# tkonolige/city2ba

Measured on AMD Instinct MI355X. Metric: million observations/sec (project+Jacobian), higher is better.
Workload: dtype f64

## Files before the change

city2ba_amd/csrc/camera_math.hpp:

```cpp
#pragma once
#include <hip/hip_runtime.h>
#include <stdint.h>
#include "pow4_libm.hpp"

namespace c2b {

#define C2B_DEV __device__ __forceinline__

constexpr int kCamBlk = 32;
constexpr int kCamHot = 24;
constexpr int kR = 0, kT = 9, kIntr = 12, kJl = 15, kCenter = 24;

constexpr int kCamGroup = 8;
__host__ __device__ inline int cam_in_group_at(int k, int j) {
    return j < 16 ? k * 16 + j : (j < 24 ? 128 + k * 8 + (j - 16) : (j < 28 ? 192 + k * 4 + (j - 24) : 224 + k * 4 + (j - 28)));
}
__host__ __device__ inline int64_t cam_group_at(int64_t c) { return (c >> 3) * (int64_t)(kCamGroup * kCamBlk); }
__host__ __device__ inline int64_t cam_light_at(int64_t c) { return cam_group_at(c) + (c & 7) * 16; }
__host__ __device__ inline int64_t cam_center_at(int64_t c) { return cam_group_at(c) + 192 + (c & 7) * 4; }
__host__ __device__ inline int64_t cam_at(int64_t c, int j) { return cam_group_at(c) + cam_in_group_at((int)(c & 7), j); }
__host__ __device__ inline int64_t cam_chunk_at(int64_t c, int j2) { return cam_at(c, 2 * j2); }
__host__ __device__ inline int64_t cam_table_doubles(int64_t n_cam) { return ((n_cam + kCamGroup - 1) / kCamGroup * kCamGroup) * (int64_t)kCamBlk; }
struct CamRec {
    const double *group; int k;
// ... 27 lines not shown
        for (int r = 0; r < 3; ++r)
            o[3 * c + r] = dot3(a[r], a[3 + r], a[6 + r], b[3 * c], b[3 * c + 1], b[3 * c + 2]);
}

template <typename T>
C2B_DEV void cm_center(const T *m, T tx, T ty, T tz, T c[3]) {
    const T m00 = m[0], m01 = m[1], m02 = m[2];
    const T m10 = m[3], m11 = m[4], m12 = m[5];
    const T m20 = m[6], m21 = m[7], m22 = m[8];
    const T det = m00 * (m11 * m22 - m21 * m12) - m10 * (m01 * m22 - m21 * m02) +
                  m20 * (m01 * m12 - m11 * m02);
    const T a0 = (m11 * m22 - m12 * m21) / det, a1 = (m12 * m20 - m10 * m22) / det,
            a2 = (m10 * m21 - m11 * m20) / det;
    const T b0 = (m21 * m02 - m22 * m01) / det, b1 = (m22 * m00 - m20 * m02) / det,
            b2 = (m20 * m01 - m21 * m00) / det;
    const T c0 = (m01 * m12 - m02 * m11) / det, c1 = (m02 * m10 - m00 * m12) / det,
            c2 = (m00 * m11 - m01 * m10) / det;
    c[0] = -dot3(a0, a1, a2, tx, ty, tz);
    c[1] = -dot3(b0, b1, b2, tx, ty, tz);
    c[2] = -dot3(c0, c1, c2, tx, ty, tz);
}

template <typename T>
C2B_DEV void cm_from_axis_angle(T ax, T ay, T az, T angle, T *o) {
    T s, c;
    sincos_t(angle, &s, &c);
    const T k = T(1.0) - c;
    o[0] = k * ax * ax + c;       o[1] = k * ax * ay + s * az;  o[2] = k * ax * az - s * ay;
    o[3] = k * ax * ay - s * az;  o[4] = k * ay * ay + c;       o[5] = k * ay * az + s * ax;
    o[6] = k * ax * az + s * ay;  o[7] = k * ay * az - s * ax;  o[8] = k * az * az + c;
}

C2B_DEV void cm_quat_from_mat(const double *m, double q[4]) {
    const double m00 = m[0], m01 = m[1], m02 = m[2], m10 = m[3], m11 = m[4], m12 = m[5],
                 m20 = m[6], m21 = m[7], m22 = m[8];
    const double trace = m00 + m11 + m22;
    double w, x, y, z, s;
    if (trace >= 0.0) {
        s = sqrt(1.0 + trace);
        w = 0.5 * s; s = 0.5 / s;
        x = (m12 - m21) * s; y = (m20 - m02) * s; z = (m01 - m10) * s;
    } else if (m00 > m11 && m00 > m22) {
        s = sqrt((m00 - m11 - m22) + 1.0);
        x = 0.5 * s; s = 0.5 / s;
        y = (m10 + m01) * s; z = (m02 + m20) * s; w = (m12 - m21) * s;
    } else if (m11 > m22) {
        s = sqrt((m11 - m00 - m22) + 1.0);
        y = 0.5 * s; s = 0.5 / s;
        z = (m21 + m12) * s; x = (m10 + m01) * s; w = (m20 - m02) * s;
    } else {
        s = sqrt((m22 - m00 - m11) + 1.0);
        z = 0.5 * s; s = 0.5 / s;
        x = (m02 + m20) * s; y = (m21 + m12) * s; w = (m01 - m10) * s;
    }
    q[0] = w; q[1] = x; q[2] = y; q[3] = z;
}

C2B_DEV void cm_mat_from_quat(const double q[4], double *o) {
    const double s = q[0], x = q[1], y = q[2], z = q[3];
    const double x2 = x + x, y2 = y + y, z2 = z + z;
    const double xx2 = x2 * x, xy2 = x2 * y, xz2 = x2 * z;
    const double yy2 = y2 * y, yz2 = y2 * z, zz2 = z2 * z;
    const double sy2 = y2 * s, sz2 = z2 * s, sx2 = x2 * s;
    o[0] = 1.0 - yy2 - zz2; o[1] = xy2 + sz2;       o[2] = xz2 - sy2;
    o[3] = xy2 - sz2;       o[4] = 1.0 - xx2 - zz2; o[5] = yz2 + sx2;
    o[6] = xz2 + sy2;       o[7] = yz2 - sx2;       o[8] = 1.0 - xx2 - yy2;
}

C2B_DEV void from_rodrigues(double w0, double w1, double w2, double *Rcm) {
    const double theta2 = dot3(w0, w1, w2, w0, w1, w2);
    if (theta2 > kEps) {
        const double angle = sqrt(theta2);
        const double inv = 1.0 / angle;
        cm_from_axis_angle(w0 * inv, w1 * inv, w2 * inv, angle, Rcm);
    } else {
        const double m[9] = {1.0, w2, -w1, -w2, 1.0, w0, w1, -w0, 1.0};
        double q[4];
        cm_quat_from_mat(m, q);
        cm_mat_from_quat(q, Rcm);
    }
}

C2B_DEV void to_rodrigues(const double *Rcm, double w[3]) {
    double q[4];
    cm_quat_from_mat(Rcm, q);
    const double angle = 2.0 * acos(q[0]);
    const double one_m = 1.0 - q[0] * q[0];
    if (one_m < kEps) {
        w[0] = w[1] = w[2] = 0.0;
    } else {
        const double d = sqrt(one_m);
        const double ax = q[1] / d, ay = q[2] / d, az = q[3] / d;
        const double inv = 1.0 / sqrt(dot3(ax, ay, az, ax, ay, az));
        w[0] = (ax * inv) * angle; w[1] = (ay * inv) * angle; w[2] = (az * inv) * angle;
    }
}

template <typename T>
C2B_DEV void transform_cam15(T *cam, const T *dRcm, T dx, T dy, T dz) {
    T c[3], v[3], nr[9];
    cm_center(cam, cam[9], cam[10], cam[11], c);
    cm_mat_vec(cam, c[0] + dx, c[1] + dy, c[2] + dz, v);
    cm_mat_mul(cam, dRcm, nr);
#pragma unroll
    for (int i = 0; i < 9; ++i) cam[i] = nr[i];
    cam[9] = T(-1.0) * v[0]; cam[10] = T(-1.0) * v[1]; cam[11] = T(-1.0) * v[2];
}

C2B_DEV void left_jacobian(double w0, double w1, double w2, double *J) {
    const double t2 = (w0 * w0 + w1 * w1) + w2 * w2;
    double a, b;
    if (t2 < 1e-2) {
        a = 0.5 + t2 * (-1.0 / 24 + t2 * (1.0 / 720 + t2 * (-1.0 / 40320 + t2 * (1.0 / 3628800))));
        b = 1.0 / 6 + t2 * (-1.0 / 120 + t2 * (1.0 / 5040 + t2 * (-1.0 / 362880 + t2 * (1.0 / 39916800))));
    } else {
        const double t = sqrt(t2);
        double sh, ch, s, c;
        sincos(0.5 * t, &sh, &ch);
        sincos(t, &s, &c);
        (void)ch; (void)c;
        a = 2.0 * sh * sh / t2;
        b = (t - s) / (t2 * t);
    }
    J[0] = 1.0 + b * (w0 * w0 - t2); J[1] = -a * w2 + b * w0 * w1;    J[2] = a * w1 + b * w0 * w2;
    J[3] = a * w2 + b * w0 * w1;     J[4] = 1.0 + b * (w1 * w1 - t2); J[5] = -a * w0 + b * w1 * w2;
    J[6] = -a * w1 + b * w0 * w2;    J[7] = a * w0 + b * w1 * w2;     J[8] = 1.0 + b * (w2 * w2 - t2);
}

C2B_DEV void fill_camblk(const double *cam15, double w0, double w1, double w2, double *blk) {
    blk[0] = cam15[0]; blk[1] = cam15[3]; blk[2] = cam15[6];
    blk[3] = cam15[1]; blk[4] = cam15[4]; blk[5] = cam15[7];
    blk[6] = cam15[2]; blk[7] = cam15[5]; blk[8] = cam15[8];
#pragma unroll
    for (int i = 0; i < 6; ++i) blk[9 + i] = cam15[9 + i];
    left_jacobian(w0, w1, w2, blk + kJl);
    double c[3];
    cm_center(cam15, cam15[9], cam15[10], cam15[11], c);
    blk[24] = c[0]; blk[25] = c[1]; blk[26] = c[2];
#pragma unroll
    for (int i = 27; i < kCamBlk; ++i) blk[i] = 0.0;
}

struct Proj {
    double qx, qy, qz;
    double px, py;
    double n, rad;
    double u, v;
};

__device__ const PowLogRow g_pow_log_tab[C2B_POW_LOG_ROWS] __attribute__((aligned(32))) = {C2B_POW_LOG_TAB};
__device__ const PowExpRow g_pow_exp_tab[C2B_POW_EXP_ROWS] __attribute__((aligned(16))) = {C2B_EXP_TAB};
C2B_DEV double pow4_libm(double x) { return pow4_glibc(x, g_pow_log_tab, g_pow_exp_tab); }

C2B_DEV void div2_shared(double a1, double a2, double b, double &q1, double &q2) {
    bool f1, f2, fd;
    const double d = __builtin_amdgcn_div_scale(a1, b, false, &fd);
    const double d2 = __builtin_amdgcn_div_scale(a2, b, false, &fd);
    double r = __builtin_amdgcn_rcp(d);
    const double e0 = fma(-d, r, 1.0);
    r = fma(r, e0, r);
    const double e1 = fma(-d, r, 1.0);
    r = fma(r, e1, r);
    const double n1 = __builtin_amdgcn_div_scale(a1, b, true, &f1);
    const double m1 = n1 * r;
    q1 = __builtin_amdgcn_div_fixup(__builtin_amdgcn_div_fmas(fma(-d, m1, n1), r, m1, f1), b, a1);
    if (__builtin_expect(__double_as_longlong(d2) == __double_as_longlong(d), 1)) {
        const double n2 = __builtin_amdgcn_div_scale(a2, b, true, &f2);
        const double m2 = n2 * r;
        q2 = __builtin_amdgcn_div_fixup(__builtin_amdgcn_div_fmas(fma(-d, m2, n2), r, m2, f2), b, a2);
    } else {
        q2 = a2 / b;
    }
}

typedef const __attribute__((address_space(3))) double *lds_cptr;
typedef const __attribute__((address_space(1))) double *glb_cptr;

template <typename P>
C2B_DEV Proj project_head(P cam, double X, double Y, double Z) {
    Proj p;
    p.qx = dot3(cam[0], cam[1], cam[2], X, Y, Z) + cam[9];
    p.qy = dot3(cam[3], cam[4], cam[5], X, Y, Z) + cam[10];
    p.qz = dot3(cam[6], cam[7], cam[8], X, Y, Z) + cam[11];
    div2_shared(-p.qx, -p.qy, p.qz, p.px, p.py);
    p.n = p.px * p.px + p.py * p.py;
    return p;
}
C2B_DEV void project_tail(Proj &p, double f, double k1, double k2, double n4) {
    p.rad = 1.0 + k1 * p.n + k2 * n4;
    const double fr = f * p.rad;
    p.u = fr * p.px;
    p.v = fr * p.py;
}
template <typename P>
C2B_DEV Proj project_obs_k0(P cam, double X, double Y, double Z) {
    Proj p = project_head(cam, X, Y, Z);
    project_tail(p, cam[12], cam[13], cam[14], p.n * p.n);
    return p;
}
template <typename P>
C2B_DEV Proj project_obs(P cam, double X, double Y, double Z) {
    Proj p = project_head(cam, X, Y, Z);
    const double k2 = cam[14];
    double n4 = p.n * p.n;
    if (k2 != 0.0) n4 = pow4_libm(sqrt(p.n));
    project_tail(p, cam[12], cam[13], k2, n4);
    return p;
}

C2B_DEV double abs_pow(double x, double norm) {
    const double a = fabs(x);
    if (norm == 2.0) return a * a;
    if (norm == 1.0) return a;
    return pow(a, norm);
}
enum { NORM_ANY = 0, NORM_1 = 1, NORM_2 = 2 };
C2B_DEV double pow_lean(double a, double y);
template <int NK>
C2B_DEV double abs_pow_k(double x, double norm) {
    const double a = fabs(x);
    if (NK == NORM_2) return a * a;
    if (NK == NORM_1) return a;
    return pow_lean(a, norm);
}

enum : uint32_t { kStreamDriftCam = 1, kStreamDriftPt = 2, kStreamNoiseCam = 3,
                  kStreamNoisePt = 4, kStreamNoiseObs = 5 };

C2B_DEV void philox4x32_10(uint32_t c0, uint32_t c1, uint32_t c2, uint32_t c3, uint32_t k0,
                           uint32_t k1, uint32_t out[4]) {
#pragma unroll
    for (int i = 0; i < 10; ++i) {
        const uint64_t p0 = (uint64_t)0xD2511F53u * c0;
        const uint64_t p1 = (uint64_t)0xCD9E8D57u * c2;
        const uint32_t n0 = (uint32_t)(p1 >> 32) ^ c1 ^ k0;
        const uint32_t n1 = (uint32_t)p1;
        const uint32_t n2 = (uint32_t)(p0 >> 32) ^ c3 ^ k1;
        const uint32_t n3 = (uint32_t)p0;
        c0 = n0; c1 = n1; c2 = n2; c3 = n3;
        k0 += 0x9E3779B9u; k1 += 0xBB67AE85u;
    }
    out[0] = c0; out[1] = c1; out[2] = c2; out[3] = c3;
}


C2B_DEV double log_unit(double x) {
    int e = __builtin_amdgcn_frexp_exp(x);
    double m = __builtin_amdgcn_frexp_mant(x);
    if (m < 0.70710678118654752440) { m = m + m; e -= 1; }
    const double f = m - 1.0, d = 2.0 + f;
    double r = __builtin_amdgcn_rcp(d);
    r = fma(fma(-d, r, 1.0), r, r);
    r = fma(fma(-d, r, 1.0), r, r);
    double q = f * r;
    q = fma(fma(-d, q, f), r, q);
    const double z = q * q, w = z * z;
    const double t1 = w * fma(w, fma(w, 1.531383769920937332e-01, 2.222219843214978396e-01), 3.999999999940941908e-01);
    const double t2 = z * fma(w, fma(w, fma(w, 1.479819860511658591e-01, 1.818357216161805012e-01), 2.857142874366239149e-01),
                              6.666666666666735130e-01);
    const double R = t2 + t1, hfsq = 0.5 * f * f, de = (double)e;
    return fma(de, 6.93147180369123816490e-01, -((hfsq - fma(q, hfsq + R, de * 1.90821492927058770002e-10)) - f));
}

C2B_DEV double exp_lean(double x) {
    const double kf = rint(x * 1.44269504088896338700e+00);
    const double hi = fma(-kf, 6.93147180369123816490e-01, x), lo = kf * 1.90821492927058770002e-10;
    const double r = hi - lo, t = r * r;
    const double c = r - t * fma(t, fma(t, fma(t, fma(t, 4.13813679705723846039e-08, -1.65339022054652515390e-06),
                                                6.61375632143793436117e-05), -2.77777777770155933842e-03), 1.66666666666666019037e-01);
    const double d = 2.0 - c;
    double q = __builtin_amdgcn_rcp(d);
    q = fma(fma(-d, q, 1.0), q, q);
    q = fma(fma(-d, q, 1.0), q, q);
    const double y = 1.0 - ((lo - (r * c) * q) - hi);
    return ldexp(y, (int)kf);
}

C2B_DEV double pow_lean(double a, double y) {
    const double l = y * log_unit(a);
    if (!(a > 0x1.0p-1000 && a < 0x1.0p+1000) || !(l > -600.0 && l < 600.0)) return pow(a, y);
    return exp_lean(l);
}

C2B_DEV double pow_t(double a, double y) { return pow_lean(a, y); }
C2B_DEV float pow_t(float a, float y) { return powf(a, y); }

C2B_DEV void sincos_kernel(double x, double &sn, double &cs) {
    const double z = x * x;
    const double ps = fma(z, fma(z, fma(z, fma(z, fma(z, 1.58969099521155010221e-10, -2.50507602534068634195e-08),
                                                  2.75573137070700676789e-06), -1.98412698298579493134e-04),
                                 8.33333333332248946124e-03), -1.66666666666666324348e-01);
    sn = fma(x * z, ps, x);
    const double pc = fma(z, fma(z, fma(z, fma(z, fma(z, -1.13596475577881948265e-11, 2.08757232129817482790e-09),
                                                  -2.75573143513906633035e-07), 2.48015872894767294178e-05),
                                 -1.38888888888741095749e-03), 4.16666666666666019037e-02);
    cs = fma(z * z, pc, fma(-0.5, z, 1.0));
}

C2B_DEV void sincos_turns(double u, double &sn, double &cs) {
    const double t = 4.0 * u, kf = rint(t);
    const int k = (int)kf;
    double s, c;
    sincos_kernel((t - kf) * 1.57079632679489661923, s, c);
    const bool swap = (k & 1) != 0;
    const double a = swap ? s : c, b = swap ? c : s;
    cs = ((k + 1) & 2) ? -a : a;
// ... 112 lines not shown
```

city2ba_amd/csrc/kernels.hpp:

```cpp
#pragma once
#include "camera_math.hpp"

namespace c2b {

constexpr int kBlock = 256;
constexpr int kWaves = kBlock / 64;
constexpr int kRedBlocks = 1024;
constexpr int kStatGrid = 512;
constexpr int kStatRec = 20;
constexpr int kStatBatch = 4;
constexpr int kStatBlock = 256;
constexpr bool kStatPipe = false;
constexpr bool kStatChunk = false;

typedef double d2_t __attribute__((ext_vector_type(2)));

C2B_DEV int64_t xcd_tile(int64_t bid, int64_t n_tiles) {
    const int64_t q = n_tiles >> 3, r = n_tiles & 7;
    const int64_t xcd = bid & 7, k = bid >> 3;
    return (xcd < r ? xcd * (q + 1) : r * (q + 1) + (xcd - r) * q) + k;
}

C2B_DEV double wave_sum(double v) {
#pragma unroll
// ... 243 lines not shown
    const int64_t i = (int64_t)blockIdx.x * blockDim.x + threadIdx.x;
    if (i >= n) return;
    double R[9], v[3];
#pragma unroll
    for (int k = 0; k < 9; ++k) R[k] = dir[9 * i + k];
    cm_mat_vec(R, pos[3 * i], pos[3 * i + 1], pos[3 * i + 2], v);
    double *o = cam15 + 15 * i;
#pragma unroll
    for (int k = 0; k < 9; ++k) o[k] = R[k];
    o[9] = -1.0 * v[0]; o[10] = -1.0 * v[1]; o[11] = -1.0 * v[2];
    o[12] = 1.0; o[13] = 0.0; o[14] = 0.0;
}

__global__ void k_points_pad(const double *__restrict__ p3, int64_t n, double4 *__restrict__ p4) {
    const int64_t i = (int64_t)blockIdx.x * blockDim.x + threadIdx.x;
    if (i >= n) return;
    p4[i] = make_double4(p3[3 * i], p3[3 * i + 1], p3[3 * i + 2], 0.0);
}
__global__ void k_points_unpad(const double4 *__restrict__ p4, int64_t n, double *__restrict__ p3) {
    const int64_t i = (int64_t)blockIdx.x * blockDim.x + threadIdx.x;
    if (i >= n) return;
    const double4 v = p4[i];
    p3[3 * i] = v.x; p3[3 * i + 1] = v.y; p3[3 * i + 2] = v.z;
}

__global__ void k_expand_rows(const uint64_t *__restrict__ row_ptr, int64_t n_cam, int64_t base,
                              int64_t n_obs, uint32_t *__restrict__ cam_idx) {
    const int64_t o = (int64_t)blockIdx.x * blockDim.x + threadIdx.x;
    if (o >= n_obs) return;
    const uint64_t key = (uint64_t)(o + base);
    int64_t lo = 0, hi = n_cam + 1;
    while (lo < hi) {
        const int64_t mid = (lo + hi) >> 1;
        if (row_ptr[mid] > key) hi = mid; else lo = mid + 1;
    }
    cam_idx[o] = (uint32_t)(lo - 1);
}

C2B_DEV uint32_t csr_search(const uint64_t *__restrict__ row_ptr, int n_cam, uint64_t o) {
    int lo = 0, hi = n_cam + 1;
    while (lo < hi) {
        const int mid = (lo + hi) >> 1;
        if (row_ptr[mid] > o) hi = mid; else lo = mid + 1;
    }
    lo = lo < 1 ? 1 : (lo > n_cam ? n_cam : lo);
    return (uint32_t)(lo - 1);
}

__global__ __launch_bounds__(256) void k_rows_pack_tiles(const uint64_t *__restrict__ row_ptr, int n_cam, int n,
                                                         uint4 *__restrict__ tiles) {
    const int tile = blockIdx.x * 256 + threadIdx.x;
    if ((int64_t)tile * 64 >= n) return;
    tiles[tile] = make_uint4(0u, 0u, csr_search(row_ptr, n_cam, (uint64_t)tile * 64), 0u);
}
__global__ __launch_bounds__(256) void k_rows_pack_marks(const uint64_t *__restrict__ row_ptr, int n_cam, int n,
                                                         uint32_t *__restrict__ tiles) {
    const int c = blockIdx.x * 256 + threadIdx.x;
    if (c >= n_cam) return;
    const uint64_t b = row_ptr[c], e = row_ptr[c + 1];
    if (e <= b || b >= (uint64_t)n || (b & 63u) == 0) return;
    uint32_t *rec = tiles + 4 * (b >> 6);
    const unsigned lane = (unsigned)(b & 63u);
    atomicOr(rec + (lane >> 5), 1u << (lane & 31u));
    if (c > 0 && row_ptr[c - 1] == b) atomicOr(rec + 2, 0x80000000u);
}

template <int OPL>
C2B_DEV void rows_cameras(const uint4 *__restrict__ tiles, const uint64_t *__restrict__ row_ptr, int n_cam, int base,
                          int n, int64_t obs_base, int lane, uint32_t (&ci)[OPL]) {
    const int last_tile = (n - 1) >> 6;
    uint4 rec[OPL];
    int tis[OPL];
#pragma unroll
    for (int t = 0; t < OPL; ++t) {
        const int ti = (base >> 6) + t;
        tis[t] = ti < last_tile ? ti : last_tile;
        rec[t] = tiles[tis[t]];
    }
#pragma unroll
    for (int t = 0; t < OPL; ++t) {
        const uint32_t lo = (rec[t].x >> 1) | (rec[t].y << 31), hi = rec[t].y >> 1;
        uint32_t c = __builtin_amdgcn_mbcnt_hi(hi, __builtin_amdgcn_mbcnt_lo(lo, rec[t].z));
        if (rec[t].z & 0x80000000u) {
            int o = tis[t] * 64 + lane;
            o = o < n ? o : n - 1;
            c = csr_search(row_ptr, n_cam, (uint64_t)(obs_base + o));
        }
        ci[t] = c;
    }
}

constexpr int kCamW = 12;


template <bool NT>
C2B_DEV void store16(char *dst, const double2 v) {
    if (NT) {
        d2_t t; t.x = v.x; t.y = v.y;
        __builtin_nontemporal_store(t, reinterpret_cast<d2_t *>(dst));
    } else {
        *reinterpret_cast<double2 *>(dst) = v;
    }
}

enum { MODE_PROJECT = 0, MODE_ERROR = 1, MODE_VISIBILITY = 2, MODE_ERROR12 = 3, MODE_NOISE_ERROR12 = 4, MODE_VISIBILITY_BITS = 5,
       MODE_RESIDUAL_KEEP = 6 };
constexpr int kObsWPB = 8;
constexpr int kCamLight = 16;

constexpr int kObsOPL = 3;

C2B_DEV int pick_cameras(uint64_t todo, uint32_t ci, int lane, uint32_t *sIdx, int &my) {
    my = -1;
    int ns = 0;
    uint64_t rest = todo;
    while (rest != 0 && ns < kCamW) {
        const uint32_t cf = __builtin_amdgcn_readlane(ci, (int)__builtin_ctzll(rest));
        const bool mine = ((rest >> lane) & 1ull) != 0 && ci == cf;
        if (mine) my = ns;
        if (lane == 0) sIdx[ns] = cf;
        rest &= ~__builtin_amdgcn_ballot_w64(mine);
        ++ns;
    }
    return ns;
}

C2B_DEV int xcd_tile32(int bid, int n_tiles) {
    const int q = n_tiles >> 3, r = n_tiles & 7;
    const int xcd = bid & 7, k = bid >> 3;
    return (xcd < r ? xcd * (q + 1) : r * (q + 1) + (xcd - r) * q) + k;
}

C2B_DEV int64_t cam_row(int64_t c, int j) {
    if (j >= kCamLight / 2) return cam_center_at(c) + 2 * (j - kCamLight / 2);
    return cam_light_at(c) + 2 * j;
}

template <int MODE, int NK = NORM_2, int OPL = kObsOPL, int WPB = kObsWPB, int MINW = 1,
          bool CSR = false, bool NTS = false, int NTL = 0>
__global__ __launch_bounds__(WPB * 64, MINW) void k_observations(
    const double *__restrict__ camblk, const double4 *__restrict__ pts4,
    const uint32_t *__restrict__ cam_idx, const uint32_t *__restrict__ pt_idx,
    const double2 *__restrict__ uv_obs, int n, int n_btiles, double norm, double max_dist,
    double2 *__restrict__ uv_out, uint8_t *__restrict__ keep, double *__restrict__ block_part,
    unsigned *__restrict__ ticket, double *__restrict__ out_sum, const uint64_t *__restrict__ row_ptr, int n_cam,
    int64_t obs_base, uint64_t seed) {
    constexpr bool VIS = MODE == MODE_VISIBILITY || MODE == MODE_VISIBILITY_BITS;
    constexpr int HOT = VIS ? 20 : kCamLight;
    constexpr int CH = HOT / 2;
    constexpr int kPerWave = 2 * kCamW * HOT + 8;
    constexpr bool POWTAB = MODE == MODE_ERROR && NK == NORM_ANY;
    constexpr int kTabN = MODE == MODE_NOISE_ERROR12 ? kNoiseTab : (POWTAB ? kPowTab : 0);
    constexpr int kTabDoubles = 2 * kTabN;
    __shared__ __attribute__((aligned(16))) double sCamAll[WPB * kPerWave + kTabDoubles];
    tab2_t *sTab = reinterpret_cast<tab2_t *>(sCamAll + WPB * kPerWave);
    constexpr int kTabTrips = (kTabN + WPB * 64 - 1) / (WPB * 64);
    tab2_t tabv[kTabTrips > 0 ? kTabTrips : 1];
    if (kTabN > 0) {
        static_assert((WPB * kPerWave) % 2 == 0, "the table's 16-byte entries start on a 16-byte boundary");
#pragma unroll
        for (int k = 0; k < kTabTrips; ++k) {
            const int i = (int)threadIdx.x + k * WPB * 64;
            tabv[k] = g_noise_tab[i < kTabN ? i : 0];
        }
    }
    const int lane = threadIdx.x & 63;
    const int wave = __builtin_amdgcn_readfirstlane(threadIdx.x >> 6);
    const int base = (xcd_tile32(blockIdx.x, n_btiles) * WPB + wave) * (OPL * 64);
    double eacc = 0.0, eacc1 = 0.0;
    if (base < n) {
        uint32_t ci[OPL], pi[OPL];
        double4 X[OPL];
#pragma unroll
        for (int t = 0; t < OPL; ++t) {
            int o = base + t * 64 + lane;
            o = o < n ? o : n - 1;
            if (!CSR) ci[t] = (NTL & 1) ? __builtin_nontemporal_load(cam_idx + o) : cam_idx[o];
            pi[t] = (NTL & 1) ? __builtin_nontemporal_load(pt_idx + o) : pt_idx[o];
        }
        if (CSR) rows_cameras<OPL>(reinterpret_cast<const uint4 *>(cam_idx), row_ptr, n_cam, base, n, 0, lane, ci);

        double *sCam = sCamAll + wave * kPerWave;
        double *sSlow = sCam + kCamW * HOT;
        uint32_t *sIdx = reinterpret_cast<uint32_t *>(sSlow + kCamW * HOT);
        const uint32_t c_first = __builtin_amdgcn_readfirstlane(ci[0]);
        const uint32_t c_last = __builtin_amdgcn_readlane(ci[OPL - 1], 63);
        uint32_t n_staged = c_last >= c_first ? c_last - c_first + 1 : 1;
        if (n_staged > (uint32_t)kCamW) n_staged = kCamW;
        constexpr int kStageTrips = (kCamW * CH + 63) / 64;
        d2_t camv[kStageTrips];
#pragma unroll
        for (int q = 0; q < kStageTrips; ++q) {
            const int ch = lane + q * 64;
            if (ch < (int)n_staged * CH) {
                const int k = ch / CH, j = ch % CH;
                camv[q] = *reinterpret_cast<const d2_t *>(camblk + cam_row((int64_t)(c_first + k), j));
            }
        }
        if (kTabN > 0) {
#pragma unroll
            for (int k = 0; k < kTabTrips; ++k) {
                const int i = (int)threadIdx.x + k * WPB * 64;
                if (i < kTabN) sTab[i] = tabv[k];
            }
        }
#pragma unroll
        for (int t = 0; t < OPL; ++t) X[t] = pts4[pi[t]];
#pragma unroll
        for (int q = 0; q < kStageTrips; ++q) {
            const int ch = lane + q * 64;
            if (ch < (int)n_staged * CH) *reinterpret_cast<d2_t *>(sCam + (ch / CH) * HOT + 2 * (ch % CH)) = camv[q];
        }
        __builtin_amdgcn_fence(__ATOMIC_RELEASE, "wavefront");
        __builtin_amdgcn_wave_barrier();
        if (kTabN > 0) __syncthreads();

#pragma unroll
        for (int t = 0; t < OPL; ++t) {
            const int tile0 = base + t * 64;
            if (tile0 >= n) break;
            const int o = tile0 + lane;
            const bool valid = o < n;
            double2 ob = make_double2(0.0, 0.0);
            if (MODE == MODE_ERROR || MODE == MODE_ERROR12 || MODE == MODE_NOISE_ERROR12 || MODE == MODE_RESIDUAL_KEEP) {
                const double2 *src = (MODE == MODE_NOISE_ERROR12 ? uv_out : uv_obs) + (valid ? o : n - 1);
                if (NTL & 2) {
                    const d2_t t2 = __builtin_nontemporal_load(reinterpret_cast<const d2_t *>(src));
                    ob = make_double2(t2.x, t2.y);
                } else {
                    ob = *src;
                }
            }
            uint32_t local = ci[t] - c_first;
            bool in = local < n_staged;
            lds_cptr cam = (lds_cptr)sCam + (in ? local : 0u) * HOT;
            Proj p = project_obs_k0(cam, X[t].x, X[t].y, X[t].z);
            uint64_t k2nz = __builtin_amdgcn_ballot_w64(cam[14] != 0.0);
            if (k2nz != 0 && ((k2nz >> lane) & 1ull)) { p.u = p.px; p.v = p.py; }
            double gx = 0.0, gy = 0.0, gz = 0.0;
            if (VIS) { gx = cam[16]; gy = cam[17]; gz = cam[18]; }
            uint64_t todo = __builtin_amdgcn_ballot_w64(valid && !in);
            while (todo != 0) {
                int my;
                __builtin_amdgcn_fence(__ATOMIC_ACQUIRE, "wavefront");
                __builtin_amdgcn_wave_barrier();
                const int ns = pick_cameras(todo, ci[t], lane, sIdx, my);
                __builtin_amdgcn_fence(__ATOMIC_RELEASE, "wavefront");
                __builtin_amdgcn_wave_barrier();
                for (int ch = lane; ch < ns * CH; ch += 64) {
                    const int k = ch / CH, j = ch % CH;
                    *reinterpret_cast<d2_t *>(sSlow + k * HOT + 2 * j) =
                        *reinterpret_cast<const d2_t *>(camblk + cam_row((int64_t)sIdx[k], j));
                }
                __builtin_amdgcn_fence(__ATOMIC_RELEASE, "wavefront");
                __builtin_amdgcn_wave_barrier();
                const bool mine = my >= 0;
                lds_cptr cam2 = (lds_cptr)sSlow + (mine ? my : 0) * HOT;
                const Proj q = project_obs_k0(cam2, X[t].x, X[t].y, X[t].z);
                const bool k2mine = mine && cam2[14] != 0.0;
                const uint64_t served = __builtin_amdgcn_ballot_w64(mine);
                k2nz = (k2nz & ~served) | __builtin_amdgcn_ballot_w64(k2mine);
                if (mine) {
                    p = q;
                    if (k2mine) { p.u = q.px; p.v = q.py; }
                    if (VIS) { gx = cam2[16]; gy = cam2[17]; gz = cam2[18]; }
                }
                todo &= ~served;
            }
            if (k2nz != 0) {
                if ((k2nz >> lane) & 1ull) {
                    Proj q;
                    q.px = p.u; q.py = p.v;
                    q.n = q.px * q.px + q.py * q.py;
                    double f, k1, k2;
                    if (valid && !in) {
                        glb_cptr g = (glb_cptr)camblk + cam_row((int64_t)ci[t], 6);
                        f = g[0]; k1 = g[1]; k2 = g[2];
                    } else {
                        f = cam[12]; k1 = cam[13]; k2 = cam[14];
                    }
                    project_tail(q, f, k1, k2, pow4_libm(sqrt(q.n)));
                    p.u = q.u; p.v = q.v;
                }
            }
            bool front = false;
            if (VIS) {
                const double dx = gx - X[t].x, dy = gy - X[t].y, dz = gz - X[t].z;
                const double dist = sqrt(dot3(dx, dy, dz, dx, dy, dz));
                front = dist < max_dist && p.qz <= 0.0;
            }
            if (VIS) {
                const bool k = front && p.u >= -1.0 && p.u <= 1.0 && p.v >= -1.0 && p.v <= 1.0;
                const double nan = __longlong_as_double(0x7ff8000000000000LL);
                if (valid) store16<NTS>(reinterpret_cast<char *>(uv_out + o), front ? make_double2(p.u, p.v) : make_double2(nan, nan));
                if (MODE == MODE_VISIBILITY_BITS) {
                    const uint64_t word = __builtin_amdgcn_ballot_w64(valid && k);
                    if (lane == 0) __builtin_nontemporal_store(word, reinterpret_cast<uint64_t *>(keep) + (tile0 >> 6));
                } else if (valid) {
                    if (NTS) __builtin_nontemporal_store((uint8_t)(k ? 1 : 0), keep + o);
                    else keep[o] = k ? 1 : 0;
                }
            } else if (MODE == MODE_PROJECT) {
                if (valid) store16<NTS>(reinterpret_cast<char *>(uv_out + o), make_double2(p.u, p.v));
            } else if (MODE == MODE_RESIDUAL_KEEP) {
                const double du = p.u - ob.x, dv = p.v - ob.y;
                const double r2 = du * du + dv * dv;
                const bool k = r2 <= norm && (!(seed & 1ull) || p.qz < 0.0);
                if (valid) {
                    if (NTS) __builtin_nontemporal_store((uint8_t)(k ? 1 : 0), keep + o);
                    else keep[o] = k ? 1 : 0;
                }
            } else if (MODE == MODE_ERROR) {
                if (POWTAB) eacc += valid ? abs_pow_tab(p.u - ob.x, norm, (lds_tab)sTab) + abs_pow_tab(p.v - ob.y, norm, (lds_tab)sTab) : 0.0;
                else eacc += valid ? abs_pow_k<NK>(p.u - ob.x, norm) + abs_pow_k<NK>(p.v - ob.y, norm) : 0.0;
            } else {
                if (MODE == MODE_NOISE_ERROR12) {
                    double c, s;
                    const double z = obs_noise_draw(seed, (uint64_t)(obs_base + (valid ? o : n - 1)), (lds_tab)sTab, c, s);
                    const double r = 0.0 + norm * z;
                    ob.x = ob.x + c * r;
                    ob.y = ob.y + s * r;
                    if (valid) store16<NTS>(reinterpret_cast<char *>(uv_out + o), ob);
                }
                const double du = p.u - ob.x, dv = p.v - ob.y;
                eacc1 += valid ? abs_pow_k<NORM_1>(du, 1.0) + abs_pow_k<NORM_1>(dv, 1.0) : 0.0;
                eacc += valid ? abs_pow_k<NORM_2>(du, 2.0) + abs_pow_k<NORM_2>(dv, 2.0) : 0.0;
            }
        }
    }
    else if (kTabN > 0) {
#pragma unroll
        for (int k = 0; k < kTabTrips; ++k) {
            const int i = (int)threadIdx.x + k * WPB * 64;
            if (i < kTabN) sTab[i] = tabv[k];
        }
        __syncthreads();
    }
    if (MODE == MODE_ERROR) ticket_fold(wave_sum(eacc), sCamAll, block_part, ticket, out_sum);
    if (MODE == MODE_ERROR12 || MODE == MODE_NOISE_ERROR12) {
        const double w[2] = {wave_sum(eacc1), wave_sum(eacc)};
        ticket_fold_n<2>(w, sCamAll, block_part, ticket, out_sum);
    }
}


template <typename P>
C2B_DEV void jacobian_obs(P cam, const double4 X, const double2 ob, double &r0, double &r1,
                          double jc[18], double jp[6]) {
    const Proj p = project_obs(cam, X.x, X.y, X.z);
    r0 = p.u - ob.x; r1 = p.v - ob.y;
    const double f = cam[12], k1 = cam[13], k2 = cam[14];
    double iz = __builtin_amdgcn_rcp(p.qz);
    iz = fma(fma(-p.qz, iz, 1.0), iz, iz);
    iz = fma(fma(-p.qz, iz, 1.0), iz, iz);
    const double s = -f * iz;
    const double c = fma(4.0 * k2, p.n, 2.0 * k1);
    const double cpx = c * p.px;
    const double B00 = fma(cpx, p.px, p.rad), B01 = cpx * p.py, B11 = fma(c * p.py, p.py, p.rad);
    const double g = fma(c, p.n, p.rad);
    const double a00 = s * B00, a01 = s * B01, a02 = s * p.px * g;
    const double a10 = s * B01, a11 = s * B11, a12 = s * p.py * g;
    const double yx = p.qx - cam[9], yy = p.qy - cam[10], yz = p.qz - cam[11];
    const double v0x = fma(yy, a02, -yz * a01), v0y = fma(yz, a00, -yx * a02), v0z = fma(yx, a01, -yy * a00);
    const double v1x = fma(yy, a12, -yz * a11), v1y = fma(yz, a10, -yx * a12), v1z = fma(yx, a11, -yy * a10);
    const P Jl = cam + kJl;
#pragma unroll
    for (int j = 0; j < 3; ++j) {
        jc[j] = fma(v0z, Jl[6 + j], fma(v0y, Jl[3 + j], v0x * Jl[j]));
        jc[9 + j] = fma(v1z, Jl[6 + j], fma(v1y, Jl[3 + j], v1x * Jl[j]));
        jp[j] = fma(a02, cam[6 + j], fma(a01, cam[3 + j], a00 * cam[j]));
        jp[3 + j] = fma(a12, cam[6 + j], fma(a11, cam[3 + j], a10 * cam[j]));
    }
    jc[3] = a00; jc[4] = a01; jc[5] = a02;
    jc[12] = a10; jc[13] = a11; jc[14] = a12;
    const double fn = f * p.n, fnn = fn * p.n;
    jc[6] = p.rad * p.px;  jc[15] = p.rad * p.py;
    jc[7] = fn * p.px;     jc[16] = fn * p.py;
    jc[8] = fnn * p.px;    jc[17] = fnn * p.py;
}

template <int NK, bool WITH_ERR, int WPB, bool NT, int OPL, int MINW, bool OBUP = true, bool CSR = false, int NTL = 0>
__global__ __launch_bounds__(WPB * 64, MINW) void k_residual_jacobian_l(
    const double *__restrict__ camblk, const double4 *__restrict__ pts4,
    const uint32_t *__restrict__ cam_idx, const uint32_t *__restrict__ pt_idx,
    const double2 *__restrict__ uv_obs, int n, int n_btiles, double norm,
    double2 *__restrict__ r_out, double *__restrict__ Jc, double *__restrict__ Jp,
    double *__restrict__ block_part, unsigned *__restrict__ ticket, double *__restrict__ out_sum,
    const uint64_t *__restrict__ row_ptr, int n_cam, int64_t obs_base) {
    constexpr int kSlab = 64 * 144 / 2;
    constexpr int kCamBytes = 2 * kCamW * kCamHot * 8 + 64;
    __shared__ __attribute__((aligned(16))) char smem[WPB * (kSlab + kCamBytes)];

    const int lane = threadIdx.x & 63;
    const int wave = __builtin_amdgcn_readfirstlane(threadIdx.x >> 6);
    const int base = (xcd_tile32(blockIdx.x, n_btiles) * WPB + wave) * (OPL * 64);
    double eacc = 0.0;
    if (base < n) {
        uint32_t ci[OPL], pi[OPL];
        double2 obs_up[OPL];
        double4 X[OPL];
#pragma unroll
        for (int t = 0; t < OPL; ++t) {
            int o = base + t * 64 + lane;
            o = o < n ? o : n - 1;
            if (!CSR) ci[t] = (NTL & 1) ? __builtin_nontemporal_load(cam_idx + o) : cam_idx[o];
            pi[t] = (NTL & 1) ? __builtin_nontemporal_load(pt_idx + o) : pt_idx[o];
            if (OBUP) {
                if (NTL & 2) {
                    const d2_t t2 = __builtin_nontemporal_load(reinterpret_cast<const d2_t *>(uv_obs + o));
                    obs_up[t] = make_double2(t2.x, t2.y);
                } else {
                    obs_up[t] = uv_obs[o];
                }
            }
        }
        if (CSR) rows_cameras<OPL>(reinterpret_cast<const uint4 *>(cam_idx), row_ptr, n_cam, base, n, obs_base, lane, ci);
#pragma unroll
        for (int t = 0; t < OPL; ++t) X[t] = pts4[pi[t]];

        char *slab = smem + wave * (kSlab + kCamBytes);
        double *sCam = reinterpret_cast<double *>(slab + kSlab);
        double *sSlow = sCam + kCamW * kCamHot;
        uint32_t *sIdx = reinterpret_cast<uint32_t *>(sSlow + kCamW * kCamHot);
        const uint32_t c_first = __builtin_amdgcn_readfirstlane(ci[0]);
        const uint32_t c_last = __builtin_amdgcn_readlane(ci[OPL - 1], 63);
        uint32_t n_staged = c_last >= c_first ? c_last - c_first + 1 : 1;
        if (n_staged > (uint32_t)kCamW) n_staged = kCamW;
        const double *cam_base = camblk + (int64_t)(c_first >> 3) * (kCamGroup * kCamBlk);
        const int c_in_group = (int)(c_first & 7u);
        for (int ch = lane; ch < (int)n_staged * (kCamHot / 2); ch += 64) {
            const int k = ch / (kCamHot / 2), j = ch % (kCamHot / 2), cg = c_in_group + k;
            const int off = (cg >> 3) * (kCamGroup * kCamBlk) + cam_in_group_at(cg & 7, 2 * j);
            *reinterpret_cast<d2_t *>(sCam + k * kCamHot + 2 * j) = *reinterpret_cast<const d2_t *>(cam_base + off);
        }
// ... 1115 lines not shown
```

city2ba_amd/csrc/pow4_libm.hpp:

```cpp
#pragma once
#include <stdint.h>
#include <string.h>
#include "pow_tables.inc"

#if defined(__HIPCC__)
#define C2B_POW_HD __host__ __device__ __forceinline__
#else
#define C2B_POW_HD static inline
#endif
#if defined(__HIP_DEVICE_COMPILE__)
#define C2B_POW_FENCE() __builtin_amdgcn_sched_barrier(0)
#else
#define C2B_POW_FENCE() ((void)0)
#endif

namespace c2b {

struct PowLogRow { uint64_t invc, logc, logctail, pad; };
struct PowExpRow { uint64_t tail, sbits; };
#define C2B_POW_LOG_ROWS 128
#define C2B_POW_EXP_ROWS 128

C2B_POW_HD double pow_asdouble(uint64_t u) {
#if defined(__HIP_DEVICE_COMPILE__)
    return __longlong_as_double((long long)u);
#else
    double d; memcpy(&d, &u, 8); return d;
#endif
}
C2B_POW_HD uint64_t pow_asuint(double d) {
#if defined(__HIP_DEVICE_COMPILE__)
    return (uint64_t)__double_as_longlong(d);
#else
    uint64_t u; memcpy(&u, &d, 8); return u;
#endif
}

C2B_POW_HD double pow_const(uint64_t bits) {
#if defined(__HIP_DEVICE_COMPILE__)
    asm volatile("" : "+s"(bits));
#endif
    return pow_asdouble(bits);
}

template <typename LT, typename ET>
C2B_POW_HD double pow4_glibc(double x, LT logtab, ET exptab) {
    uint64_t ix = pow_asuint(x);
    uint32_t topx = (uint32_t)(ix >> 52);
    if (topx - 1u > 0x7fdu) {
        if (2 * ix - 1 >= 2 * 0x7ff0000000000000ULL - 1) return x * x;
        if (ix >> 63) { ix &= 0x7fffffffffffffffULL; topx &= 0x7ffu; }
        if (topx == 0) {
            ix = pow_asuint(pow_asdouble(ix) * 0x1p52);
            ix &= 0x7fffffffffffffffULL;
            ix -= 52ULL << 52;
        }
    }
    const uint64_t tmp = ix - 0x3fe6955500000000ULL;
    const int i = (int)((tmp >> 45) & 127);
    const int k = (int)((int64_t)tmp >> 52);
    const uint64_t iz = ix - (tmp & 0xfff0000000000000ULL);
    const double z = pow_asdouble(iz), kd = (double)k;
    const double invc = pow_asdouble(logtab[i].invc), logc = pow_asdouble(logtab[i].logc), logctail = pow_asdouble(logtab[i].logctail);
    const double r = __builtin_fma(z, invc, -1.0);
    C2B_POW_FENCE();
    const double t1 = __builtin_fma(kd, pow_const(C2B_POW_LN2HI), logc);
    const double lo1 = __builtin_fma(kd, pow_const(C2B_POW_LN2LO), logctail);
    C2B_POW_FENCE();
    const double t2 = r + t1;
    const double lo2 = (t1 - t2) + r;
    const double s12 = lo1 + lo2;
    C2B_POW_FENCE();
    const double ar = r * pow_const(C2B_POW_A0);
    const double ar2 = r * ar;
    const double lo3 = __builtin_fma(ar, r, -ar2);
    const double s123 = s12 + lo3;
    C2B_POW_FENCE();
    const double hi = t2 + ar2;
    const double lo4 = (t2 - hi) + ar2;
    const double s1234 = s123 + lo4;
    C2B_POW_FENCE();
    const double q3 = __builtin_fma(r, pow_const(C2B_POW_A6), pow_const(C2B_POW_A5));
    const double q2 = __builtin_fma(r, pow_const(C2B_POW_A4), pow_const(C2B_POW_A3));
    const double q23 = __builtin_fma(q3, ar2, q2);
    C2B_POW_FENCE();
    const double q1 = __builtin_fma(r, pow_const(C2B_POW_A2), pow_const(C2B_POW_A1));
    const double qq = __builtin_fma(ar2, q23, q1);
    const double ar3 = r * ar2;
    const double lo = __builtin_fma(ar3, qq, s1234);
    C2B_POW_FENCE();
    const double lhi = hi + lo;
    const double ltail = (hi - lhi) + lo;
    const double y = 4.0;
    const double ehi = y * lhi;
    const double elo = __builtin_fma(y, ltail, __builtin_fma(lhi, y, -ehi));
    C2B_POW_FENCE();
    const uint64_t ebits = pow_asuint(ehi);
    uint32_t abstop = (uint32_t)(ebits >> 52) & 0x7ffu;
    if (abstop - 0x3c9u > 0x3eu) {
        if ((int32_t)(abstop - 0x3c9u) < 0) return 1.0 + ehi;
        if (abstop > 0x408u) return (ebits >> 63) ? 0.0 : pow_asdouble(0x7ff0000000000000ULL);
        abstop = 0;
    }
    const double shift = pow_const(C2B_EXP_SHIFT);
    double kd2 = __builtin_fma(ehi, pow_const(C2B_EXP_INVLN2N), shift);
    const uint64_t ki = pow_asuint(kd2);
    kd2 = kd2 - shift;
    double rr = __builtin_fma(kd2, pow_const(C2B_EXP_NEGLN2HIN), ehi);
    rr = __builtin_fma(kd2, pow_const(C2B_EXP_NEGLN2LON), rr);
    const int idx = (int)(ki & 127);
    uint64_t sbits = exptab[idx].sbits + (ki << 45);
    rr = elo + rr;
    C2B_POW_FENCE();
    const double p23 = __builtin_fma(rr, pow_const(C2B_EXP_C3), pow_const(C2B_EXP_C2));
    const double tr = rr + pow_asdouble(exptab[idx].tail);
    const double r2 = rr * rr;
    const double s1 = __builtin_fma(p23, r2, tr);
    C2B_POW_FENCE();
    const double p45 = __builtin_fma(rr, pow_const(C2B_EXP_C5), pow_const(C2B_EXP_C4));
    const double r4 = r2 * r2;
    const double tm = __builtin_fma(p45, r4, s1);
    C2B_POW_FENCE();
    if (abstop == 0) {
        if ((ki & 0x80000000ULL) == 0) {
            sbits -= 1009ULL << 52;
            const double sc = pow_asdouble(sbits);
            return 0x1p1009 * __builtin_fma(sc, tm, sc);
        }
        sbits += 1022ULL << 52;
        const double sc = pow_asdouble(sbits);
        const double st = tm * sc;
        double yy = sc + st;
        if (__builtin_fabs(yy) < 1.0) {
            const double one = yy < 0.0 ? -1.0 : 1.0;
            const double l0 = (sc - yy) + st;
            const double h1 = yy + one;
            const double l1 = ((one - h1) + yy) + l0;
            yy = (l1 + h1) - one;
            if (yy == 0.0) yy = pow_asdouble(sbits & 0x8000000000000000ULL);
        }
        return 0x1p-1022 * yy;
    }
    const double scale = pow_asdouble(sbits);
    return __builtin_fma(tm, scale, scale);
}

}
```

Before: 27770.

## Stage packed pow lookup tables in LDS and drop scheduling fences

Packs the glibc-style pow log table (dropping the unused fourth column) and exp table into one constant array. In observation kernels that have no other shared table, each wave copies it into LDS when any lane may need the k2 distortion path, and pow4 then reads its tables from LDS instead of global memory. The LDS variant also compiles without the sched_barrier fences, letting the scheduler interleave the pow arithmetic. This costs extra LDS per workgroup (asserted to still fit four workgroups per CU) and a per-wave copy plus ballot.

```diff
diff --git a/city2ba_amd/csrc/camera_math.hpp b/city2ba_amd/csrc/camera_math.hpp
--- a/city2ba_amd/csrc/camera_math.hpp
+++ b/city2ba_amd/csrc/camera_math.hpp
@@ -203,6 +203,12 @@
 __device__ const PowExpRow g_pow_exp_tab[C2B_POW_EXP_ROWS] __attribute__((aligned(16))) = {C2B_EXP_TAB};
 C2B_DEV double pow4_libm(double x) { return pow4_glibc(x, g_pow_log_tab, g_pow_exp_tab); }
 
+__device__ const PowPack g_pow_pack = pow_pack_make();
+typedef uint64_t u64x2_t __attribute__((ext_vector_type(2)));
+typedef const __attribute__((address_space(3))) uint64_t *lds_u64;
+typedef PowLogPacked<lds_u64> PowLogLds;
+typedef PowExpPacked<lds_u64> PowExpLds;
+
 C2B_DEV void div2_shared(double a1, double a2, double b, double &q1, double &q2) {
     bool f1, f2, fd;
     const double d = __builtin_amdgcn_div_scale(a1, b, false, &fd);
diff --git a/city2ba_amd/csrc/kernels.hpp b/city2ba_amd/csrc/kernels.hpp
--- a/city2ba_amd/csrc/kernels.hpp
+++ b/city2ba_amd/csrc/kernels.hpp
@@ -419,7 +419,10 @@
     constexpr bool POWTAB = MODE == MODE_ERROR && NK == NORM_ANY;
     constexpr int kTabN = MODE == MODE_NOISE_ERROR12 ? kNoiseTab : (POWTAB ? kPowTab : 0);
     constexpr int kTabDoubles = 2 * kTabN;
-    __shared__ __attribute__((aligned(16))) double sCamAll[WPB * kPerWave + kTabDoubles];
+    constexpr bool PLDS = kTabN == 0;
+    constexpr int kPowAt = WPB * kPerWave + kTabDoubles;
+    __shared__ __attribute__((aligned(16))) double sCamAll[kPowAt + (PLDS ? kPowPackWords : 0)];
+    static_assert(sizeof(sCamAll) <= 40960, "four workgroups per CU");
     tab2_t *sTab = reinterpret_cast<tab2_t *>(sCamAll + WPB * kPerWave);
     constexpr int kTabTrips = (kTabN + WPB * 64 - 1) / (WPB * 64);
     tab2_t tabv[kTabTrips > 0 ? kTabTrips : 1];
@@ -481,6 +484,25 @@
         __builtin_amdgcn_fence(__ATOMIC_RELEASE, "wavefront");
         __builtin_amdgcn_wave_barrier();
         if (kTabN > 0) __syncthreads();
+
+        if (PLDS) {
+            bool mayk2 = lane < (int)n_staged && ((lds_cptr)sCam)[lane * HOT + 14] != 0.0;
+#pragma unroll
+            for (int t = 0; t < OPL; ++t) mayk2 = mayk2 || ci[t] - c_first >= n_staged;
+            if (__builtin_amdgcn_ballot_w64(mayk2) != 0) {
+                constexpr int kPowTrips = kPowPackWords / 2 / 64;
+                static_assert(kPowTrips * 128 == kPowPackWords, "whole trips of 64 chunks of 16 bytes");
+                const u64x2_t *src = reinterpret_cast<const u64x2_t *>(g_pow_pack.w);
+                u64x2_t *dst = reinterpret_cast<u64x2_t *>(sCamAll + kPowAt);
+                u64x2_t pv[kPowTrips];
+#pragma unroll
+                for (int k = 0; k < kPowTrips; ++k) pv[k] = src[lane + 64 * k];
+#pragma unroll
+                for (int k = 0; k < kPowTrips; ++k) dst[lane + 64 * k] = pv[k];
+                __builtin_amdgcn_fence(__ATOMIC_RELEASE, "wavefront");
+                __builtin_amdgcn_wave_barrier();
+            }
+        }
 
 #pragma unroll
         for (int t = 0; t < OPL; ++t) {
@@ -546,7 +568,14 @@
                     } else {
                         f = cam[12]; k1 = cam[13]; k2 = cam[14];
                     }
-                    project_tail(q, f, k1, k2, pow4_libm(sqrt(q.n)));
+                    double n4;
+                    if (PLDS) {
+                        const lds_u64 tab = (lds_u64)reinterpret_cast<const uint64_t *>(sCamAll + kPowAt);
+                        n4 = pow4_glibc<false>(sqrt(q.n), PowLogLds{tab}, PowExpLds{tab + kPowPackLog});
+                    } else {
+                        n4 = pow4_libm(sqrt(q.n));
+                    }
+                    project_tail(q, f, k1, k2, n4);
                     p.u = q.u; p.v = q.v;
                 }
             }
diff --git a/city2ba_amd/csrc/pow4_libm.hpp b/city2ba_amd/csrc/pow4_libm.hpp
--- a/city2ba_amd/csrc/pow4_libm.hpp
+++ b/city2ba_amd/csrc/pow4_libm.hpp
@@ -5,11 +5,13 @@
 
 #if defined(__HIPCC__)
 #define C2B_POW_HD __host__ __device__ __forceinline__
+#define C2B_POW_HD_M __host__ __device__ __forceinline__
 #else
 #define C2B_POW_HD static inline
+#define C2B_POW_HD_M inline
 #endif
 #if defined(__HIP_DEVICE_COMPILE__)
-#define C2B_POW_FENCE() __builtin_amdgcn_sched_barrier(0)
+#define C2B_POW_FENCE() do { if (FENCED) __builtin_amdgcn_sched_barrier(0); } while (0)
 #else
 #define C2B_POW_FENCE() ((void)0)
 #endif
@@ -20,6 +22,31 @@
 struct PowExpRow { uint64_t tail, sbits; };
 #define C2B_POW_LOG_ROWS 128
 #define C2B_POW_EXP_ROWS 128
+
+constexpr int kPowPackLog = 3 * C2B_POW_LOG_ROWS;
+constexpr int kPowPackWords = kPowPackLog + 2 * C2B_POW_EXP_ROWS;
+struct alignas(16) PowPack { uint64_t w[kPowPackWords]; };
+constexpr PowPack pow_pack_make() {
+    constexpr uint64_t lg[4 * C2B_POW_LOG_ROWS] = {C2B_POW_LOG_TAB};
+    constexpr uint64_t ex[2 * C2B_POW_EXP_ROWS] = {C2B_EXP_TAB};
+    PowPack p{};
+    for (int i = 0; i < C2B_POW_LOG_ROWS; ++i)
+        for (int k = 0; k < 3; ++k) p.w[3 * i + k] = lg[4 * i + k];
+    for (int i = 0; i < 2 * C2B_POW_EXP_ROWS; ++i) p.w[kPowPackLog + i] = ex[i];
+    return p;
+}
+template <typename P>
+struct PowLogPacked {
+    P p;
+    struct Row { uint64_t invc, logc, logctail; };
+    C2B_POW_HD_M Row operator[](int i) const { const P r = p + 3 * i; return Row{r[0], r[1], r[2]}; }
+};
+template <typename P>
+struct PowExpPacked {
+    P p;
+    struct Row { uint64_t tail, sbits; };
+    C2B_POW_HD_M Row operator[](int i) const { const P r = p + 2 * i; return Row{r[0], r[1]}; }
+};
 
 C2B_POW_HD double pow_asdouble(uint64_t u) {
 #if defined(__HIP_DEVICE_COMPILE__)
@@ -43,7 +70,7 @@
     return pow_asdouble(bits);
 }
 
-template <typename LT, typename ET>
+template <bool FENCED = true, typename LT, typename ET>
 C2B_POW_HD double pow4_glibc(double x, LT logtab, ET exptab) {
     uint64_t ix = pow_asuint(x);
     uint32_t topx = (uint32_t)(ix >> 52);
```

Result: no change. 27970, median of 5 (+0.7%).
